# jgrodzki/radix_sort

Measured on AMD Instinct MI355X. Metric: Gkeys/sec (u64), higher is better.
Workload: dtype u64

## Files before the change

include/rsx.h:

```cpp
#ifndef RSX_H
#define RSX_H

#include <stddef.h>
#include <stdint.h>

#ifdef __cplusplus
extern "C" {
#endif

#define RSX_VERSION 200

enum {
    RSX_OK = 0,
    RSX_ERR_ARG = -1,
    RSX_ERR_UNSUPPORTED = -2,
    RSX_ERR_HIP = -3,
    RSX_ERR_NOMEM = -4,
    RSX_ERR_NODEVICE = -5,
    RSX_ERR_WORKSPACE = -6,
    RSX_ERR_INTERNAL = -7
};

enum {
    RSX_KEY_UNSIGNED = 0,
    RSX_KEY_SIGNED = 1,
    RSX_KEY_FLOAT = 2
};

#define RSX_MAX_ELEM_BYTES 32768u
typedef struct rsx_layout {
    uint32_t elem_bytes;
    uint32_t key_offset;
    uint32_t key_bytes;
    uint32_t key_kind;
} rsx_layout;

typedef struct rsx_ctx rsx_ctx;

int rsx_ctx_create(int device, rsx_ctx **out);
int rsx_ctx_destroy(rsx_ctx *ctx);
int rsx_ctx_reserve(rsx_ctx *ctx, size_t n, const rsx_layout *layout);
int rsx_ctx_check(rsx_ctx *ctx, void *stream);
enum {
    RSX_OPT_TILE_SCHEDULE = 1,
    RSX_OPT_RANKING = 2,
    RSX_OPT_STATUS_SCOPE = 3,
    RSX_OPT_XCD_MAJOR = 4,
    RSX_OPT_BYTE_COUNTING = 5,
    RSX_OPT_MAX_REGIONS = 6,
    RSX_OPT_HOT_LANES = 7,
    RSX_OPT_VERBOSE = 8,
    RSX_OPT_RANK_CHECK = 9,
    RSX_OPT_SMALL_SORT = 10,
    RSX_OPT_MID_SORT = 11      ,
    RSX_OPT_WIDE_SORT = 12,
    RSX_OPT_BUCKET_SKIP = 13,
    RSX_OPT_BUCKET_GROUP = 14
};
int rsx_ctx_set_option(rsx_ctx *ctx, int option, uint64_t value);
enum {
    RSX_INFO_RANK_ATOMIC = 1,
    RSX_INFO_L2_LOCAL = 2,
    RSX_INFO_NUM_CU = 3,
    RSX_INFO_DEVICE = 4,
    RSX_INFO_LAST_PASSES = 5,
    RSX_INFO_LAST_PAIRS = 6
};
int rsx_ctx_get_info(rsx_ctx *ctx, int what, uint64_t *out);
enum { RSX_PROF_HIST = 0, RSX_PROF_SCAN = 1, RSX_PROF_SWEEP = 2, RSX_PROF_OTHER = 3, RSX_PROF_KINDS = 4 };
int rsx_ctx_profile(rsx_ctx *ctx, int enable);
int rsx_ctx_profile_read(rsx_ctx *ctx, double *ms, uint64_t *launches);
const char *rsx_last_error(const rsx_ctx *ctx);
const char *rsx_strerror(int status);
int rsx_version(void);

int rsx_sort_device(rsx_ctx *ctx, void *d_data, void *d_tmp, size_t n, const rsx_layout *layout,
                    void *stream);

int rsx_sort_host(rsx_ctx *ctx, void *data, size_t n, const rsx_layout *layout);

int rsx_sort_segments_device(rsx_ctx *ctx, void *d_data, void *d_tmp, size_t n, const rsx_layout *layout,
                             const uint64_t *d_offsets, size_t nseg, uint64_t max_seg_len, void *stream);
int rsx_sort_rows_device(rsx_ctx *ctx, void *d_data, void *d_tmp, size_t rows, size_t row_len,
                         const rsx_layout *layout, void *stream);
#define RSX_SEG_CLASSES 2
int rsx_segment_caps(const rsx_layout *layout, uint32_t *caps);

enum { RSX_ORDER_ASCENDING = 0, RSX_ORDER_DESCENDING = 1 };

int rsx_sort_pairs_device(rsx_ctx *ctx, void *d_keys, void *d_values, size_t n, uint32_t key_bytes,
                          uint32_t key_kind, uint32_t value_bytes, int order, void *stream);
int rsx_argsort_device(rsx_ctx *ctx, const void *d_keys, void *d_index, size_t n, uint32_t key_bytes,
                       uint32_t key_kind, uint32_t index_bytes, int order, void *stream);
int rsx_ctx_reserve_pairs(rsx_ctx *ctx, size_t n, uint32_t key_bytes, uint32_t value_bytes);

int rsx_histogram_device(rsx_ctx *ctx, const void *d_src, size_t n, const rsx_layout *layout,
                         uint32_t digit, uint64_t *d_hist, void *stream);
int rsx_partition_device(rsx_ctx *ctx, const void *d_src, void *d_dst, size_t n,
                         const rsx_layout *layout, uint32_t digit, uint64_t *d_hist, void *stream);
int rsx_partition_count_device(rsx_ctx *ctx, const void *d_src, size_t n, const rsx_layout *layout, uint32_t digit,
                               uint32_t nsub, uint64_t *d_hist, void *stream);
int rsx_partition_scatter_device(rsx_ctx *ctx, const void *d_src, void *d_dst, size_t n, const rsx_layout *layout,
                                 uint32_t digit, uint32_t nsub, uint32_t k, void *stream);

int rsx_segmented_copy_device(rsx_ctx *ctx, const void *d_src, void *d_dst, uint32_t elem_bytes,
                              const uint64_t *d_src_off, const uint64_t *d_dst_off,
                              const uint64_t *d_len, uint32_t nseg, void *stream);

int rsx_bounds_device(rsx_ctx *ctx, const void *d_sorted, size_t n, const rsx_layout *layout,
                      const uint64_t *d_queries, uint32_t nq, uint64_t *d_out, void *stream);
// ... 36 lines not shown
```

radix_sort_amd/__init__.py:

```python
from .api import (PRIMITIVES, Context, RadixDigits, default_context, digits_of, radix_argsort, radix_sort, radix_sort_pairs,
                  radix_sort_rows, radix_sort_segments, radix_sort_sharded, segment_caps, tuple_of)
from ._lib import (GEN_CONSTANT, GEN_GEOMETRIC, GEN_PAYLOAD_ZERO, GEN_REVERSED, GEN_SORTED, GEN_STEP, GEN_UNIFORM,
                   GEN_ZIPF, INFO_L2_LOCAL, INFO_LAST_PAIRS, INFO_LAST_PASSES, INFO_RANK_ATOMIC, KEY_FLOAT, KEY_SIGNED, KEY_UNSIGNED, OPT_BYTE_COUNTING,
                   OPT_HOT_LANES, OPT_MAX_REGIONS, OPT_MID_SORT, OPT_WIDE_SORT, OPT_BUCKET_SKIP, OPT_BUCKET_GROUP, OPT_RANK_CHECK, OPT_RANKING, OPT_SMALL_SORT, OPT_STATUS_SCOPE, OPT_TILE_SCHEDULE, OPT_VERBOSE,
                   OPT_XCD_MAJOR, SHARD_EXCHANGE_FIRST, SHARD_SORT_FIRST, Layout, RsxError)

__all__ = ["radix_sort", "radix_sort_pairs", "radix_argsort", "radix_sort_segments", "radix_sort_rows", "segment_caps", "radix_sort_sharded", "RadixDigits", "PRIMITIVES", "tuple_of", "digits_of", "Context", "default_context",
           "Layout", "RsxError", "KEY_UNSIGNED", "KEY_SIGNED", "KEY_FLOAT", "GEN_UNIFORM", "GEN_ZIPF", "GEN_STEP",
           "GEN_SORTED", "GEN_REVERSED", "GEN_CONSTANT", "GEN_GEOMETRIC", "GEN_PAYLOAD_ZERO", "OPT_TILE_SCHEDULE",
           "OPT_RANKING", "OPT_STATUS_SCOPE", "OPT_XCD_MAJOR", "OPT_BYTE_COUNTING", "OPT_MAX_REGIONS", "OPT_HOT_LANES",
           "OPT_VERBOSE", "OPT_RANK_CHECK", "OPT_SMALL_SORT", "OPT_MID_SORT", "OPT_WIDE_SORT", "OPT_BUCKET_SKIP", "OPT_BUCKET_GROUP", "INFO_RANK_ATOMIC", "INFO_L2_LOCAL", "INFO_LAST_PASSES", "INFO_LAST_PAIRS", "SHARD_EXCHANGE_FIRST", "SHARD_SORT_FIRST"]
```

radix_sort_amd/_lib.py:

```python
from __future__ import annotations

import ctypes
import os

from . import _build

SYMBOLS = [
    "rsx_ctx_create", "rsx_ctx_destroy", "rsx_ctx_reserve", "rsx_ctx_check", "rsx_ctx_set_option", "rsx_ctx_get_info",
    "rsx_ctx_profile", "rsx_ctx_profile_read", "rsx_last_error",
    "rsx_strerror", "rsx_version", "rsx_sort_device", "rsx_sort_host", "rsx_histogram_device",
    "rsx_partition_device", "rsx_partition_count_device", "rsx_partition_scatter_device", "rsx_splitter_count_device",
    "rsx_splitter_pick_device", "rsx_segmented_copy_device", "rsx_bounds_device", "rsx_bounds_ranges_device", "rsx_sort_sharded",
    "rsx_sort_sharded_ex", "rsx_generate_device", "rsx_verify_device",
    "rsx_sort_segments_device", "rsx_sort_rows_device", "rsx_segment_caps",
    "rsx_sort_pairs_device", "rsx_argsort_device", "rsx_ctx_reserve_pairs",
]
SEG_CLASSES = 2

OK, ERR_ARG, ERR_UNSUPPORTED, ERR_HIP, ERR_NOMEM, ERR_NODEVICE, ERR_WORKSPACE, ERR_INTERNAL = 0, -1, -2, -3, -4, -5, -6, -7
KEY_UNSIGNED, KEY_SIGNED, KEY_FLOAT = 0, 1, 2
PROF_HIST, PROF_SCAN, PROF_SWEEP, PROF_OTHER, PROF_KINDS = 0, 1, 2, 3, 4
GEN_UNIFORM, GEN_ZIPF, GEN_STEP, GEN_SORTED, GEN_REVERSED, GEN_CONSTANT, GEN_GEOMETRIC = 0, 1, 2, 3, 4, 5, 6
GEN_PAYLOAD_ZERO = 0x100
(OPT_TILE_SCHEDULE, OPT_RANKING, OPT_STATUS_SCOPE, OPT_XCD_MAJOR, OPT_BYTE_COUNTING, OPT_MAX_REGIONS, OPT_HOT_LANES,
 OPT_VERBOSE, OPT_RANK_CHECK, OPT_SMALL_SORT, OPT_MID_SORT, OPT_WIDE_SORT, OPT_BUCKET_SKIP, OPT_BUCKET_GROUP) = 1, 2, 3, 4, 5, 6, 7, 8, 9, 10, 11, 12, 13, 14
INFO_RANK_ATOMIC, INFO_L2_LOCAL, INFO_NUM_CU, INFO_DEVICE, INFO_LAST_PASSES, INFO_LAST_PAIRS = 1, 2, 3, 4, 5, 6
ORDER_ASCENDING, ORDER_DESCENDING = 0, 1
SHARD_EXCHANGE_FIRST, SHARD_SORT_FIRST = 0, 1


class Layout(ctypes.Structure):
    _fields_ = [
        ("elem_bytes", ctypes.c_uint32),
        ("key_offset", ctypes.c_uint32),
        ("key_bytes", ctypes.c_uint32),
        ("key_kind", ctypes.c_uint32),
    ]

    def __repr__(self):
        return f"Layout(elem_bytes={self.elem_bytes}, key_offset={self.key_offset}, key_bytes={self.key_bytes}, key_kind={self.key_kind})"


class RsxError(RuntimeError):
    def __init__(self, status: int, msg: str):
        super().__init__(f"rsx status {status}: {msg}")
        self.status = status


_LIB = None


def lib_path() -> str:
    return os.environ.get("RSX_LIBRARY") or _build.LIB


def load():
    global _LIB
    if _LIB is not None:
        return _LIB
    try:
        import torch
    except ImportError:
        pass
    path = lib_path()
    if not os.path.exists(path):
        raise ImportError(
            f"{path} is missing: build it with `python -m radix_sort_amd._build` "
            "(needs hipcc); there is no CPU fallback for the sort path")
    L = ctypes.CDLL(path)
    vp, sz, lp = ctypes.c_void_p, ctypes.c_size_t, ctypes.POINTER(Layout)
    u32, u64, i = ctypes.c_uint32, ctypes.c_uint64, ctypes.c_int
    L.rsx_ctx_create.argtypes = [i, ctypes.POINTER(vp)]
    L.rsx_ctx_destroy.argtypes = [vp]
    L.rsx_ctx_reserve.argtypes = [vp, sz, lp]
    L.rsx_ctx_check.argtypes = [vp, vp]
    L.rsx_ctx_set_option.argtypes = [vp, i, u64]
    L.rsx_ctx_get_info.argtypes = [vp, i, ctypes.POINTER(ctypes.c_uint64)]
    L.rsx_ctx_profile.argtypes = [vp, i]
# ... 34 lines not shown
```

radix_sort_amd/csrc/rsx.hip:

```cpp
#include "rsx_internal.hpp"
#include "rsx_misc_kernels.hpp"
#include "rsx_any_kernels.hpp"

#include <cmath>

using namespace rsx;
using namespace rsxh;

namespace {

bool layout_ok(const rsx_layout* L, bool any_width = false) {
    if (!L) return false;
    const uint32_t kb = L->key_bytes;
    if (any_width ? (kb < 1 || kb > 16) : !(kb == 1 || kb == 2 || kb == 4 || kb == 8 || kb == 16)) return false;
    if (L->key_kind > RSX_KEY_FLOAT) return false;
    if (L->key_kind == RSX_KEY_FLOAT && !(kb == 4 || kb == 8)) return false;
    if (L->elem_bytes == 0 || (uint64_t)L->key_offset + kb > L->elem_bytes) return false;
    return true;
}
const EsLaunchers* launchers_for(uint32_t es) {
    switch (es) {
        case 1: return &es_launchers<1>();
        case 2: return &es_launchers<2>();
        case 4: return &es_launchers<4>();
// ... 760 lines not shown
        case RSX_OPT_TILE_SCHEDULE:
            if (value > 1) return fail(ctx, RSX_ERR_ARG, "RSX_OPT_TILE_SCHEDULE: 0 (roll call) or 1 (tickets)");
            flag(OPT_DYNAMIC_TILES, value == 1);
            return RSX_OK;
        case RSX_OPT_RANKING:
            if (value > 2) return fail(ctx, RSX_ERR_ARG, "RSX_OPT_RANKING: 0 (auto), 1 (ballots) or 2 (LDS atomics)");
            flag(OPT_BALLOT_RANKS, value == 1);
            flag(OPT_ATOMIC_RANKS, value == 2);
            return RSX_OK;
        case RSX_OPT_STATUS_SCOPE:
            if (value > 1) return fail(ctx, RSX_ERR_ARG, "RSX_OPT_STATUS_SCOPE: 0 (auto) or 1 (agent)");
            flag(OPT_AGENT_STATUS, value == 1);
            return RSX_OK;
        case RSX_OPT_XCD_MAJOR:
            if (value > 1) return fail(ctx, RSX_ERR_ARG, "RSX_OPT_XCD_MAJOR: 0 or 1");
            flag(OPT_NO_XCD_MAJOR, value == 0);
            return RSX_OK;
        case RSX_OPT_BYTE_COUNTING:
            if (value > 1) return fail(ctx, RSX_ERR_ARG, "RSX_OPT_BYTE_COUNTING: 0 or 1");
            flag(OPT_GENERAL_BYTES, value == 0);
            return RSX_OK;
        case RSX_OPT_MAX_REGIONS:
            if (value > (uint64_t)MAX_REGIONS) return fail(ctx, RSX_ERR_ARG, "RSX_OPT_MAX_REGIONS: 0 (default) .. 32");
            ctx->max_regions = (uint32_t)value;
            return RSX_OK;
        case RSX_OPT_HOT_LANES:
            if (value < 2 || value > 65) return fail(ctx, RSX_ERR_ARG, "RSX_OPT_HOT_LANES: 2 .. 65");
            ctx->hot_lanes = (uint32_t)value;
            return RSX_OK;
        case RSX_OPT_VERBOSE:
            flag(OPT_VERBOSE, value != 0);
            return RSX_OK;
        case RSX_OPT_RANK_CHECK:
            flag(OPT_RANK_CHECK, value != 0);
            return RSX_OK;
        case RSX_OPT_SMALL_SORT:
            if (value > 1) return fail(ctx, RSX_ERR_ARG, "RSX_OPT_SMALL_SORT: 0 or 1");
            flag(OPT_NO_SMALL_SORT, value == 0);
            return RSX_OK;
        case RSX_OPT_WIDE_SORT:
            if (value > 3) return fail(ctx, RSX_ERR_ARG, "RSX_OPT_WIDE_SORT: 0 (off), 1 (auto), 2 (always) or 3 (auto from 2^22 elements on)");
            ctx->wide_mode = (uint32_t)value;
            ctx->wide_skip = 0;
            if (ctx->host_err) host_word(ctx, HV_WIDE_HINT) = 0;
            return RSX_OK;
        case RSX_OPT_BUCKET_SKIP:
            if (value > 1) return fail(ctx, RSX_ERR_ARG, "RSX_OPT_BUCKET_SKIP: 0 or 1");
            ctx->bucket_no_skip = value == 0 ? 1u : 0u;
            return RSX_OK;
        case RSX_OPT_BUCKET_GROUP:
            if (value > 1) return fail(ctx, RSX_ERR_ARG, "RSX_OPT_BUCKET_GROUP: 0 or 1");
            ctx->bucket_group = (uint32_t)value;
            return RSX_OK;
        case RSX_OPT_MID_SORT:
            if (value > 3) return fail(ctx, RSX_ERR_ARG, "RSX_OPT_MID_SORT: 0 (off), 1 (forecast), 2 (always split) or 3 (always LSD passes)");
            flag(OPT_NO_MID_SORT, value == 0);
            ctx->mid_force = value >= 2 ? (uint32_t)value - 1u : 0u;
            return RSX_OK;
        default:
            return fail(ctx, RSX_ERR_ARG, "unknown option");
    }
} catch (...) {
    return RSX_ERR_NOMEM;
}

int rsx_ctx_get_info(rsx_ctx* ctx, int what, uint64_t* out) try {
    if (!ctx || !out) return RSX_ERR_ARG;
    std::lock_guard<std::mutex> lk(ctx->mu);
    DeviceGuard g(ctx->device);
    if (what == RSX_INFO_RANK_ATOMIC || what == RSX_INFO_L2_LOCAL) {
        int rc = ensure_aux(ctx, nullptr);
        if (rc) return rc;
    }
    switch (what) {
        case RSX_INFO_RANK_ATOMIC: *out = ctx->rank_atomic ? 1 : 0; return RSX_OK;
        case RSX_INFO_L2_LOCAL: *out = ctx->l2_local ? 1 : 0; return RSX_OK;
        case RSX_INFO_NUM_CU: *out = (uint64_t)ctx->num_cu; return RSX_OK;
        case RSX_INFO_DEVICE: *out = (uint64_t)ctx->device; return RSX_OK;
        case RSX_INFO_LAST_PASSES: {
            if (ctx->last_path == 6) {
                *out = (uint64_t)(ctx->last_sort_passes & 0xFFu) | (uint64_t)6 << 24;
                return RSX_OK;
            }
            *out = (uint64_t)ctx->last_path << 24 | (uint64_t)ctx->last_route << 28;
            if (!ctx->aux || ctx->last_sort_passes == 0) return RSX_OK;
            if (ctx->busy) RSX_HIP(hipEventSynchronize(ctx->last_event));
            uint64_t stat = 0, placed = 0;
            uint32_t path = ctx->last_path, passes = ctx->last_sort_passes;
            if (path == 5 && ctx->wide_buf) {
                uint32_t verdict = 0;
                RSX_HIP(hipMemcpy(&verdict, reinterpret_cast<char*>(ctx->wide_buf) + WIDE_PLAN_OFFSET, sizeof verdict, hipMemcpyDeviceToHost));
                if ((verdict & VERDICT_PATH_MASK) == VERDICT_HYBRID) passes = 2;
                else path = 0;
            }
            for (uint32_t p = 0; p < passes && p < (uint32_t)MAX_PASSES; ++p) {
                uint32_t mode = 0;
                RSX_HIP(hipMemcpy(&mode, reinterpret_cast<uint32_t*>(cb_of(ctx, ctx->cb_last) + CB_TICKETS) + (size_t)p * TICKET_WORDS + ROLL_MODE,
                                  sizeof mode, hipMemcpyDeviceToHost));
                stat += (mode == 1u || mode == 3u) ? 1u : 0u;
                placed += mode == 3u ? 1u : 0u;
            }
            *out = (uint64_t)passes | (stat << 8) | (placed << 16) | ((uint64_t)path << 24) | ((uint64_t)ctx->last_route << 28);
            return RSX_OK;
        }
        case RSX_INFO_LAST_PAIRS: *out = (uint64_t)ctx->last_pairs; return RSX_OK;
        default: return fail(ctx, RSX_ERR_ARG, "unknown info id");
// ... 910 lines not shown
```

radix_sort_amd/csrc/rsx_internal.hpp:

```cpp
#pragma once
#include "rsx_device.hpp"

#include <hip/hip_runtime.h>

#include <cstdio>
#include <cstdlib>
#include <cstring>
#include <mutex>
#include <new>
#include <algorithm>
#include <string>
#include <thread>
#include <utility>
#include <vector>

#include "../../include/rsx.h"

namespace rsxh {
using namespace rsx;

constexpr int MAX_PASSES = 16;
constexpr size_t J_BYTES = (size_t)J_REPL * MAX_REGIONS * RADIX * sizeof(uint64_t);
constexpr size_t TICKET_WORDS = ROLL_SHARDS + (size_t)ROLL_SHARD_COUNT * ROLL_SHARD_STRIDE;
constexpr uint32_t PART_MAX_SUB = 16;
constexpr uint32_t MID_MAX_REGIONS = 16;
constexpr size_t CB_TICKETS = 0;
constexpr size_t CB_JT = ((MAX_PASSES * TICKET_WORDS * 4 + 255) / 256) * 256;
constexpr size_t JT_BYTES = (size_t)J_REPL * MID_MAX_REGIONS * RADIX * sizeof(uint64_t);
constexpr size_t CB_J0 = CB_JT + JT_BYTES;
constexpr size_t CB_BYTES = CB_J0 + J_BYTES;
static_assert(CB_BYTES % 16 == 0, "control blocks are zeroed with 16-byte stores");
constexpr int CB_COUNT = 3;
constexpr size_t OFF_J1 = CB_COUNT * CB_BYTES;
constexpr size_t OFF_J2 = OFF_J1 + J_BYTES;
constexpr size_t OFF_PART_TICKETS = OFF_J2 + J_BYTES;
constexpr size_t OFF_BASE = OFF_PART_TICKETS + ((TICKET_WORDS * 4 + 255) / 256) * 256;
constexpr size_t OFF_FLAGS = OFF_BASE + 4096;
constexpr size_t OFF_DBG = OFF_FLAGS + 256;
constexpr size_t AUX_BYTES = OFF_DBG + 1024;
constexpr uint32_t HV_ERROR = 0, HV_MID_HINT = 8, HV_WIDE_HINT = 9;

enum : uint32_t {
    OPT_DYNAMIC_TILES = 1u << 0,
    OPT_BALLOT_RANKS = 1u << 1,
    OPT_ATOMIC_RANKS = 1u << 2,
    OPT_AGENT_STATUS = 1u << 3,
    OPT_NO_XCD_MAJOR = 1u << 4,
    OPT_GENERAL_BYTES = 1u << 5,
    OPT_VERBOSE = 1u << 6,
    OPT_RANK_CHECK = 1u << 7,
    OPT_NO_SMALL_SORT = 1u << 8,
    OPT_NO_MID_SORT = 1u << 9,
};

}

struct rsx_ctx {
    int device = 0;
    std::mutex mu;
    std::string err = "";
    void* status = nullptr;
    size_t status_bytes = 0;
    char* aux = nullptr;
    uint32_t* host_err = nullptr;
    uint32_t* host_err_dev = nullptr;
    void* host_buf[2] = {nullptr, nullptr};
    size_t host_bytes = 0;
    hipStream_t copy_stream = nullptr;
    void* pinned[4] = {nullptr, nullptr, nullptr, nullptr};
    hipEvent_t copy_event[4] = {nullptr, nullptr, nullptr, nullptr};
    uint32_t wide_skip = 0;
    char* wide_buf = nullptr;
    uint32_t wide_mode = 1;
    std::vector<const void*> lds_attr;
    uint64_t wide_tried_sig = 0, wide_refused_sig = 0;
    uint32_t bucket_no_skip = 0;
    uint32_t bucket_group = 1;
    uint32_t* ovf16 = nullptr;
    unsigned long long* part_J = nullptr;
    hipStream_t shard_stream = nullptr;
    uint64_t* shard_q = nullptr;
    uint64_t* shard_out = nullptr;
    uint64_t* shard_hist = nullptr;
    uint64_t* shard_host = nullptr;
    std::vector<uint64_t> shard_stage;
    int num_cu = 256;
    uint32_t last_path = 0;
    uint32_t last_sort_passes = 0;
    uint32_t last_route = 0;
    char* any_buf = nullptr;
    size_t any_bytes = 0;
    uint32_t last_pairs = 0;
    uint64_t cb_used[2][2] = {{0, 0}, {0, 0}};
    uint32_t cb_alt = 0;
    uint32_t cb_last = 0;
    bool cb_dirty = false;
    uint32_t mid_choice = 0;
    uint32_t mid_force = 0;
    uint32_t mid_cooldown = 0;
    bool rank_atomic = false;
    bool l2_local = false;
    uint32_t hot_lanes = 16;
    uint32_t options = 0;
    uint32_t max_regions = 0;
    uint32_t dbg = 0;
    hipStream_t last_stream = nullptr;
    hipEvent_t last_event = nullptr;
    bool busy = false;
    bool prof = false;
    std::vector<std::pair<hipEvent_t, hipEvent_t>> prof_pending[RSX_PROF_KINDS];
    std::vector<std::pair<hipEvent_t, hipEvent_t>> prof_free;
    double prof_ms[RSX_PROF_KINDS] = {0, 0, 0, 0};
    uint64_t prof_n[RSX_PROF_KINDS] = {0, 0, 0, 0};
    std::vector<float> prof_each;
};

namespace rsxh {

struct SortRun {
    uint32_t cb = 0;
    CleanList clean = {{nullptr, nullptr, nullptr}, {0, 0, 0}};
    Gate gate = {nullptr, 0, 0};
    const DigitSpec* spec_dev = nullptr;
    uint32_t* tickets_override = nullptr;
};
struct SweepPass {
    uint32_t index;
    bool last;
    uint32_t mid;
};
// ... 200 lines not shown
```

radix_sort_amd/csrc/rsx_launch_impl.hpp:

```cpp
#pragma once
#include <cstdlib>
#include "rsx_internal.hpp"
#include "rsx_small_kernel.hpp"
#include "rsx_mid_kernels.hpp"
#include "rsx_segment_kernels.hpp"

#ifndef RSX_HIST_BLOCKS_PER_CU
#define RSX_HIST_BLOCKS_PER_CU 8
#endif

namespace rsxh {

inline uint32_t rank_atomic_of(const rsx_ctx* ctx) { return (ctx->rank_atomic && !(ctx->options & OPT_BALLOT_RANKS)) ? 1u : 0u; }
constexpr CleanList CLEAN_NONE = {{nullptr, nullptr, nullptr}, {0, 0, 0}};

inline uint64_t hist_blocks_per_region(const rsx_ctx* ctx, const RegionGeom& g) {
    const uint64_t per_block = 512ull * 16;
    uint64_t bpr = ((1ull << g.region_shift) + per_block - 1) / per_block;
    const uint64_t cap = ((uint64_t)ctx->num_cu * RSX_HIST_BLOCKS_PER_CU + g.num_regions - 1) / g.num_regions;
    if (bpr > cap) bpr = cap;
    return bpr == 0 ? 1 : bpr;
}
template <int ES, bool FLT>
int launch_hist_t(rsx_ctx* ctx, SortRun& run, const void* src, const RegionGeom& g, const rsx_layout* L, uint32_t digit,
// ... 333 lines not shown
            auto kern = rsx_count16top_kernel<ES, true>;
            ensure_lds(ctx, reinterpret_cast<const void*>(kern), 131072);
            hipLaunchKernelGGL(kern, dim3(parts), dim3(1024), 131072, st, static_cast<const Elem<ES>*>(src), (uint64_t)n, plan, make_xform(L), P,
                               ctx->ovf16, region_shift, k);
        } else {
            auto kern = rsx_count16top_kernel<ES, false>;
            ensure_lds(ctx, reinterpret_cast<const void*>(kern), 131072);
            hipLaunchKernelGGL(kern, dim3(parts), dim3(1024), 131072, st, static_cast<const Elem<ES>*>(src), (uint64_t)n, plan, make_xform(L), P,
                               ctx->ovf16, region_shift, k);
        }
        RSX_HIP(hipGetLastError());
        return RSX_OK;
    }
}

template <int ES>
int launch_marginal16(rsx_ctx* ctx, SortRun& run, const uint32_t* P, uint32_t parts, uint32_t k, const RegionGeom& g, unsigned long long* J,
                      unsigned long long* jclear, hipStream_t st) {
    const uint64_t zero16_n = status_rows(g) * RADIX * (status32(g) ? 4u : 8u) / 16u;
    uint32_t grid = (uint32_t)ctx->num_cu * 8u;
    if (grid < parts) grid = parts;
    LaunchTimer lt(ctx, RSX_PROF_HIST, st);
    hipLaunchKernelGGL(rsx_marginal16_kernel<ES>, dim3(grid), dim3(256), 0, st, P, parts, k, g, J, jclear, status32(g) ? 1u : 0u,
                       static_cast<uint4*>(ctx->status), zero16_n, run.clean, run.gate);
    RSX_HIP(hipGetLastError());
    run.clean = CLEAN_NONE;
    return RSX_OK;
}

template <int ES>
int launch_bucket16(rsx_ctx* ctx, const SortRun& run, void* data, void* scratch, size_t n, const rsx_layout* L, const uint64_t* starts,
                    const WidePlan* plan, hipStream_t st) {
    if constexpr (ES < 4) {
        return fail(ctx, RSX_ERR_INTERNAL, "launch_bucket16: narrow elements");
    } else {
        constexpr int KPT = bucket_kpt_for(ES);
        if (L->key_bytes < 4) return fail(ctx, RSX_ERR_INTERNAL, "launch_bucket16: key width out of range");
        SmallArgs a = small_args(ctx, L, L->key_bytes - 2, L->key_bytes, false);
        a.src = data;
        a.data = data;
        a.cap = bucket_cap(ES);
        LaunchTimer lt(ctx, RSX_PROF_OTHER, st);
        const uint64_t avg = (uint64_t)n / 65536u;
        const uint32_t gs = group_shift(ctx, n, L);
        const Gate base = run.gate;
        auto go = [&](auto wgc, auto kc, uint32_t form, uint32_t group_shift) {
            constexpr int WGS = decltype(wgc)::value;
            constexpr int K = decltype(kc)::value;
            SmallArgs b = a;
            b.group_shift = group_shift;
            if (group_shift) b.passes = L->key_bytes;
            static_assert(cape<ES, K, WGS>() == bucket_cape(ES, K, WGS), "host and device agree on what a workgroup holds");
            const size_t lds = (size_t)cape<ES, K, WGS>() * ES + (WGS / 64) * RADIX * bucket_cnt_bytes() + 64 + 3 * RADIX * sizeof(uint32_t);
            auto kern = rsx_bucket16_kernel<ES, K, WGS>;
            ensure_lds(ctx, reinterpret_cast<const void*>(kern), lds);
            int per_cu = (int)((size_t)163840 / lds);
            if (per_cu < 1) per_cu = 1;
            if (per_cu > 4 * RSX_B16_WAVES(WGS) * 64 / WGS) per_cu = 4 * RSX_B16_WAVES(WGS) * 64 / WGS;
            const Gate g{base.word, VERDICT_PATH_MASK | VERDICT_FORM_MASK, VERDICT_HYBRID | form};
            hipLaunchKernelGGL(kern, dim3((uint32_t)(ctx->num_cu * per_cu)), dim3(WGS), lds, st, b, starts, scratch, plan, g);
        };
        using std::integral_constant;
        constexpr int KBIG = wide_kpt_for(ES);
        if (gs >= 2) go(integral_constant<int, 512>{}, integral_constant<int, KPT>{}, VERDICT_GROUPS, gs);
        if (avg <= (uint64_t)256 * KPT) go(integral_constant<int, 256>{}, integral_constant<int, KPT>{}, VERDICT_WG256, 0);
        if (avg <= (uint64_t)512 * KPT) go(integral_constant<int, 512>{}, integral_constant<int, KPT>{}, VERDICT_WG512, 0);
        const bool big_form = KBIG != KPT && wide_big_form(ES, n);
        if (big_form) go(integral_constant<int, 1024>{}, integral_constant<int, KBIG>{}, VERDICT_WG1024, 0);
        else go(integral_constant<int, 1024>{}, integral_constant<int, KPT>{}, VERDICT_WG1024, 0);
        {
            constexpr int KMED = medium_kpt_for(ES);
            const size_t lds = (size_t)cape<ES, KMED, 1024>() * ES + 16 * RADIX * bucket_cnt_bytes() + 64 + 3 * RADIX * sizeof(uint32_t);
            auto kern = rsx_bucket16_medium_kernel<ES, KMED, 1024>;
            ensure_lds(ctx, reinterpret_cast<const void*>(kern), lds);
            const Gate g{base.word, VERDICT_PATH_MASK | VERDICT_MEDIUM, VERDICT_HYBRID | VERDICT_MEDIUM};
            hipLaunchKernelGGL(kern, dim3((uint32_t)ctx->num_cu), dim3(1024), lds, st, a, starts, scratch, plan, (uint32_t)(256 * KPT), (uint32_t)(512 * KPT),
                               (uint32_t)(big_form ? cape<ES, KBIG, 1024>() : cape<ES, KPT, 1024>()), g);
        }
        RSX_HIP(hipGetLastError());
        return RSX_OK;
    }
}

template <int ES>
int launch_segcopy(rsx_ctx* ctx, const void* src, void* dst, const uint64_t* so, const uint64_t* dof,
                   const uint64_t* len, uint32_t nseg, hipStream_t st) {
    const uint32_t bps = 8;
    hipLaunchKernelGGL((rsx_segcopy_kernel<ES>), dim3(nseg * bps), dim3(256), 0, st,
                       static_cast<const Elem<ES>*>(src), static_cast<Elem<ES>*>(dst), so, dof, len, nseg, bps);
    RSX_HIP(hipGetLastError());
    return RSX_OK;
}

template <int ES>
int launch_segment_sort(rsx_ctx* ctx, void* data, void* tmp, size_t n, const rsx_layout* L, const uint64_t* offsets, uint64_t nseg,
                        uint64_t row_len, uint64_t max_len, uint32_t* launched, hipStream_t st) {
    constexpr int KPT = bucket_kpt_for(ES);
    constexpr uint32_t CAP0 = cape<ES, KPT, 256>(), CAP1 = cape<ES, KPT, 1024>();
    static_assert(CAP0 == segment_cap(ES, 0) && CAP1 == segment_cap(ES, 1), "host and device agree on what a workgroup holds");
    if (L->key_bytes > 16) return fail(ctx, RSX_ERR_INTERNAL, "launch_segment_sort: key width out of range");
    SmallArgs a = small_args(ctx, L, L->key_bytes, L->key_bytes, true);
    if (L->key_bytes < 6) a.no_skip = 1u;
    SmallArgs am = a;
    am.map_load = am.map_store = 0;
    for (uint32_t d = 0; d < L->key_bytes; ++d) am.spec[d] = make_spec(L, d);
    SegArgs s;
    std::memset(&s, 0, sizeof s);
// ... 50 lines not shown
```

radix_sort_amd/csrc/rsx_small_kernel.hpp:

```cpp
#pragma once
#include "rsx_device.hpp"

namespace rsx {

struct SmallArgs {
    const void* src;
    void* data;
    uint32_t n;
    uint32_t passes;
    uint32_t rank_atomic;
    uint32_t map_load;
    uint32_t map_store;
    DigitSpec spec[16];
    KeyXform xf;
    const uint32_t* top_tot;
    uint32_t cap;
    uint32_t no_skip;
    uint32_t group_shift;
    uint32_t key_offset, key_bytes;
    uint32_t* hint;
};

struct PassPlan {
    uint32_t first, end;
// ... 396 lines not shown
    for (int w = 0; w < ES / 4; ++w) {
        mm.hi[w] = pp.mask[w];
        mm.lo[w] = pp.low[w];
    }
    return mend_listed<ES>(reinterpret_cast<Elem<ES>*>(smem), mend_count<ES, KPT, WG>(smem), s_flag, n, (uint32_t)WG, ties, mm) != 0;
}
template <int ES, int KPT, int WG>
__device__ __forceinline__ void local_store_regs(const SmallArgs& a, Elem<ES>* __restrict__ dst, const uint32_t n, Elem<ES> (&x)[KPT]) {
#pragma unroll
    for (int j = 0; j < KPT; ++j) {
        const uint32_t i = (uint32_t)j * WG + threadIdx.x;
        if (i < n) {
            if (a.map_store) key_map<ES, true>(x[j], a.xf);
            dst[i] = x[j];
        }
    }
}

template <int ES, int KPT, int WG>
__device__ __forceinline__ bool local_finish(const SmallArgs& a, Elem<ES>* __restrict__ dst, const uint32_t n, unsigned char* smem, const PassPlan& pp,
                                             uint32_t* s_flag) {
    Elem<ES> x[KPT];
    uint32_t ties;
    if (!local_check<ES, KPT, WG>(pp, n, smem, x, ties)) {
        local_store_regs<ES, KPT, WG>(a, dst, n, x);
        return true;
    }
    if (!local_mend_listed<ES, KPT, WG>(n, smem, pp, s_flag, ties)) return false;
    local_store<ES, KPT, WG>(a, dst, n, smem);
    return true;
}

template <int ES, int KPT, int WG>
__device__ __forceinline__ void local_sort_skip(const SmallArgs& a, const Elem<ES>* __restrict__ src, Elem<ES>* __restrict__ dst, const uint32_t n,
                                                unsigned char* smem, PassPlan& pp, uint32_t* s_flag) {
    using E = Elem<ES>;
    E e[KPT];
    local_load<ES, KPT, WG>(a, src, n, e);
    local_passes<ES, KPT, WG>(a, e, n, smem, pp.first, pp.end);
    if (pp.first == 0) {
        local_store<ES, KPT, WG>(a, dst, n, smem);
    } else if (!local_finish<ES, KPT, WG>(a, dst, n, smem, pp, s_flag)) {
        pp.first = 0;
        const uint32_t kp = (n + WG - 1) / WG, seg = (threadIdx.x >> 6) * (WAVE * kp) + (threadIdx.x & 63u);
#pragma unroll
        for (int j = 0; j < KPT; ++j)
            if ((uint32_t)j < kp) e[j] = reinterpret_cast<const E*>(smem)[seg + (uint32_t)j * WAVE];
        __syncthreads();
        local_passes<ES, KPT, WG>(a, e, n, smem, 0, pp.end);
        local_store<ES, KPT, WG>(a, dst, n, smem);
    }
}

template <int ES, int KPT>
__global__ __launch_bounds__(512) void rsx_small_sort_kernel(const SmallArgs a) {
    extern __shared__ __attribute__((aligned(16))) unsigned char smem[];
    local_sort<ES, KPT, 512>(a, static_cast<const Elem<ES>*>(a.src), static_cast<Elem<ES>*>(a.data), a.n, smem);
}

template <int ES, int KPT, int WG>
__global__ __launch_bounds__(WG) void rsx_bucket_sort_kernel(const SmallArgs a) {
    extern __shared__ __attribute__((aligned(16))) unsigned char smem[];
    uint64_t* s_red = reinterpret_cast<uint64_t*>(smem);
    const uint32_t tid = threadIdx.x, v = blockIdx.x;
    uint64_t c = 0;
    if (tid < RADIX) {
        c = a.top_tot[tid];
        if (tid == v) s_red[4] = c;
        if (v == 0) {
            uint64_t big = c;
#pragma unroll
            for (int o = 32; o > 0; o >>= 1) {
                const uint64_t y = __shfl_xor(big, o);
                big = y > big ? y : big;
            }
            if ((tid & 63u) == 0u) s_red[5 + (tid >> 6)] = big;
        }
        uint64_t below = tid < v ? c : 0ull;
#pragma unroll
        for (int o = 32; o > 0; o >>= 1) below += __shfl_xor(below, o);
        if ((tid & 63u) == 0u) s_red[tid >> 6] = below;
    }
    __syncthreads();
    const uint64_t start = s_red[0] + s_red[1] + s_red[2] + s_red[3];
    const uint64_t count = s_red[4];
    if (v == 0 && tid == 0) {
        uint64_t big = s_red[5];
        for (int w = 1; w < 4; ++w) big = s_red[5 + w] > big ? s_red[5 + w] : big;
        __hip_atomic_store(a.hint, big <= (uint64_t)a.cap / 4 ? 1u : big <= (uint64_t)a.cap ? 3u : 2u, __ATOMIC_RELAXED, __HIP_MEMORY_SCOPE_SYSTEM);
    }
    __syncthreads();
    if (count == 0) return;
    if (count > (uint64_t)cape<ES, KPT, WG>()) {
        big_bucket_sort<ES, KPT, WG>(a, const_cast<Elem<ES>*>(static_cast<const Elem<ES>*>(a.src)) + start,
                                     static_cast<Elem<ES>*>(a.data) + start, (uint32_t)count, smem);
        return;
    }
    if constexpr (ES < 8) {
        local_sort<ES, KPT, WG>(a, static_cast<const Elem<ES>*>(a.src) + start, static_cast<Elem<ES>*>(a.data) + start, (uint32_t)count, smem);
    } else {
        PassPlan pp;
        pp.end = a.passes;
        pp.first = a.no_skip ? 0u : first_digit_for((uint32_t)count, 8u * a.passes, a.passes);
        pp.set_masks(a.key_offset, a.key_bytes);
        uint32_t* s_flag = reinterpret_cast<uint32_t*>(reinterpret_cast<typename WaveCnt<ES>::T*>(smem + (size_t)cape<ES, KPT, WG>() * sizeof(Elem<ES>)) + (WG / WAVE) * RADIX) + (WG / WAVE);
        local_sort_skip<ES, KPT, WG>(a, static_cast<const Elem<ES>*>(a.src) + start, static_cast<Elem<ES>*>(a.data) + start, (uint32_t)count, smem, pp,
                                     s_flag);
    }
}

template <int ES, int KPT, int WG>
__global__ __launch_bounds__(WG, RSX_B16_WAVES(WG)) void rsx_bucket16_kernel(const SmallArgs a, const uint64_t* __restrict__ starts, void* scratch,
                                                                         const WidePlan* __restrict__ plan, Gate gate) {
    extern __shared__ __attribute__((aligned(16))) unsigned char smem[];
    if (!gate_open(gate)) return;
    using E = Elem<ES>;
    constexpr int NWAVE = WG / WAVE;
    uint32_t* s_flag = reinterpret_cast<uint32_t*>(reinterpret_cast<typename WaveCnt<ES>::T*>(smem + (size_t)cape<ES, KPT, WG>() * sizeof(E)) + NWAVE * RADIX) + NWAVE;
    const uint32_t gs = a.group_shift != 0 ? plan->group_shift : 0;
    const bool medium = (plan->verdict & VERDICT_MEDIUM) != 0;
    PassPlan pp;
    pp.end = gs == 0 ? plan->pass_end : plan->group_end;
    if (pp.end == 0) {
        if (a.map_store) {
            const uint64_t n = starts[65536];
            E* data = static_cast<E*>(a.data);
            for (uint64_t i = (uint64_t)blockIdx.x * WG + threadIdx.x; i < n; i += (uint64_t)gridDim.x * WG) {
                E x = data[i];
                key_map<ES, true>(x, a.xf);
                data[i] = x;
            }
        }
        return;
    }
    const uint32_t b_lo = plan->window_top - 15u;
    const uint32_t end_sub = pp.end;
    if (gs != 0) pp.end = (b_lo + gs + 7u) / 8u;
    {
        const uint64_t big = (uint64_t)plan->scan_max << gs;
        const uint32_t m = big < (uint64_t)cape<ES, KPT, WG>() ? (uint32_t)big : cape<ES, KPT, WG>();
        pp.first = a.no_skip ? 0u : first_digit_for(m, b_lo + gs, pp.end);
    }
    pp.set_masks(a.key_offset, a.key_bytes);
    for (uint32_t g = blockIdx.x; g < (65536u >> gs); g += gridDim.x) {
        const uint32_t b0 = g << gs;
        const uint64_t gstart = starts[b0];
        const uint64_t gcount = starts[b0 + (1u << gs)] - gstart;
        if (gcount == 0) continue;
        const bool whole = gs == 0 || gcount <= (uint64_t)cape<ES, KPT, WG>();
        const uint32_t nsub = whole ? 1u : 1u << gs;
        for (uint32_t sub = 0; sub < nsub; ++sub) {
            uint64_t start = gstart, count = gcount;
            if (!whole) {
                start = starts[b0 + sub];
                count = starts[b0 + sub + 1] - start;
            }
            if (count != 0) {
                E* bucket = static_cast<E*>(a.data) + start;
                if (count <= (uint64_t)cape<ES, KPT, WG>()) {
                    const uint32_t first = pp.first, end = pp.end;
                    if (!whole) {
                        pp.first = 0;
                        pp.end = end_sub;
                    }
                    local_sort_skip<ES, KPT, WG>(a, bucket, bucket, (uint32_t)count, smem, pp, s_flag);
                    if (!whole) {
                        pp.first = first;
                        pp.end = end;
                    }
                } else if (!medium) {
                    big_bucket_sort<ES, KPT, WG>(a, bucket, static_cast<E*>(scratch) + start, (uint32_t)count, smem);
                }
            }
            __syncthreads();
        }
    }
}

template <int ES, int KPT, int WG>
__global__ __launch_bounds__(WG, RSX_B16_WAVES(WG)) void rsx_bucket16_medium_kernel(const SmallArgs a, const uint64_t* __restrict__ starts, void* scratch,
                                                                                const WidePlan* __restrict__ plan, uint32_t cap256, uint32_t cap512,
                                                                                uint32_t cap1024, Gate gate) {
    extern __shared__ __attribute__((aligned(16))) unsigned char smem[];
    __shared__ uint32_t s_part[2];
    if (!gate_open(gate)) return;
    using E = Elem<ES>;
    constexpr int NWAVE = WG / WAVE;
    constexpr uint32_t CAPE = cape<ES, KPT, WG>();
    uint32_t* s_flag = reinterpret_cast<uint32_t*>(reinterpret_cast<typename WaveCnt<ES>::T*>(smem + (size_t)CAPE * sizeof(E)) + NWAVE * RADIX) + NWAVE;
    const uint32_t tid = threadIdx.x;
    const uint32_t form = plan->verdict & VERDICT_FORM_MASK;
    const uint64_t handled = form == VERDICT_WG256 ? cap256 : form == VERDICT_WG1024 ? cap1024 : cap512;
    const uint32_t end = plan->pass_end;
    if (end == 0) return;
    const uint32_t b_lo = plan->window_top - 15u;
    for (uint32_t b = blockIdx.x; b < 65536u; b += gridDim.x) {
        const uint64_t start = starts[b];
        const uint64_t count = starts[b + 1] - start;
        if (count <= handled) continue;
        E* bucket = static_cast<E*>(a.data) + start;
        E* scr = static_cast<E*>(scratch) + start;
        uint32_t k = 0;
        while (k < 8u && (count >> k) > (uint64_t)CAPE * 6u / 10u) ++k;
        if (k > b_lo) k = b_lo;
        const bool split = !(k == 0 || (count >> k) > (uint64_t)CAPE || count > 0xFFFFFFFFull);
        uint32_t kmask = 0, part_start = 0, part_count = (uint32_t)count;
        PassPlan pp;
        pp.end = end;
        pp.first = 0;
        if (split) {
            DigitSpec sp{};
            const uint32_t ebit = 8u * a.key_offset + b_lo - k;
            sp.word = ebit >> 5;
            sp.shift = ebit & 31u;
            kmask = (1u << k) - 1u;
            part_start = part_count = 0;
            const uint32_t km = kmask;
            stream_pass<ES, KPT, WG>(a, bucket, scr, (uint32_t)count, smem, [&](const E& x) { return elem_digit_any<ES>(x, sp) & km; }, false, part_start,
// ... 32 lines not shown
```

Before: 67.97.

## Prefetch next bucket into LDS during store in bucket16 kernel

Adds a prefetching variant of the 16-bit bucket sort kernel that issues asynchronous global-to-LDS loads of the next bucket this workgroup will handle. The loads are interleaved with the store of the current sorted bucket, and the next local sort reads its input from LDS instead of global memory. The goal is to hide global load latency between consecutive buckets. In exchange it adds inline assembly, alignment and bounds conditions, and a waitcnt on every bucket. The variant is on by default for 1024-thread workgroups with 8- or 16-byte elements.

```diff
diff --git a/include/rsx.h b/include/rsx.h
--- a/include/rsx.h
+++ b/include/rsx.h
@@ -55,7 +55,8 @@
     RSX_OPT_MID_SORT = 11      ,
     RSX_OPT_WIDE_SORT = 12,
     RSX_OPT_BUCKET_SKIP = 13,
-    RSX_OPT_BUCKET_GROUP = 14
+    RSX_OPT_BUCKET_GROUP = 14,
+    RSX_OPT_BUCKET_PREFETCH = 15
 };
 int rsx_ctx_set_option(rsx_ctx *ctx, int option, uint64_t value);
 enum {
diff --git a/radix_sort_amd/__init__.py b/radix_sort_amd/__init__.py
--- a/radix_sort_amd/__init__.py
+++ b/radix_sort_amd/__init__.py
@@ -2,11 +2,11 @@
                   radix_sort_rows, radix_sort_segments, radix_sort_sharded, segment_caps, tuple_of)
 from ._lib import (GEN_CONSTANT, GEN_GEOMETRIC, GEN_PAYLOAD_ZERO, GEN_REVERSED, GEN_SORTED, GEN_STEP, GEN_UNIFORM,
                    GEN_ZIPF, INFO_L2_LOCAL, INFO_LAST_PAIRS, INFO_LAST_PASSES, INFO_RANK_ATOMIC, KEY_FLOAT, KEY_SIGNED, KEY_UNSIGNED, OPT_BYTE_COUNTING,
-                   OPT_HOT_LANES, OPT_MAX_REGIONS, OPT_MID_SORT, OPT_WIDE_SORT, OPT_BUCKET_SKIP, OPT_BUCKET_GROUP, OPT_RANK_CHECK, OPT_RANKING, OPT_SMALL_SORT, OPT_STATUS_SCOPE, OPT_TILE_SCHEDULE, OPT_VERBOSE,
+                   OPT_HOT_LANES, OPT_MAX_REGIONS, OPT_MID_SORT, OPT_WIDE_SORT, OPT_BUCKET_SKIP, OPT_BUCKET_GROUP, OPT_BUCKET_PREFETCH, OPT_RANK_CHECK, OPT_RANKING, OPT_SMALL_SORT, OPT_STATUS_SCOPE, OPT_TILE_SCHEDULE, OPT_VERBOSE,
                    OPT_XCD_MAJOR, SHARD_EXCHANGE_FIRST, SHARD_SORT_FIRST, Layout, RsxError)
 
 __all__ = ["radix_sort", "radix_sort_pairs", "radix_argsort", "radix_sort_segments", "radix_sort_rows", "segment_caps", "radix_sort_sharded", "RadixDigits", "PRIMITIVES", "tuple_of", "digits_of", "Context", "default_context",
            "Layout", "RsxError", "KEY_UNSIGNED", "KEY_SIGNED", "KEY_FLOAT", "GEN_UNIFORM", "GEN_ZIPF", "GEN_STEP",
            "GEN_SORTED", "GEN_REVERSED", "GEN_CONSTANT", "GEN_GEOMETRIC", "GEN_PAYLOAD_ZERO", "OPT_TILE_SCHEDULE",
            "OPT_RANKING", "OPT_STATUS_SCOPE", "OPT_XCD_MAJOR", "OPT_BYTE_COUNTING", "OPT_MAX_REGIONS", "OPT_HOT_LANES",
-           "OPT_VERBOSE", "OPT_RANK_CHECK", "OPT_SMALL_SORT", "OPT_MID_SORT", "OPT_WIDE_SORT", "OPT_BUCKET_SKIP", "OPT_BUCKET_GROUP", "INFO_RANK_ATOMIC", "INFO_L2_LOCAL", "INFO_LAST_PASSES", "INFO_LAST_PAIRS", "SHARD_EXCHANGE_FIRST", "SHARD_SORT_FIRST"]
+           "OPT_VERBOSE", "OPT_RANK_CHECK", "OPT_SMALL_SORT", "OPT_MID_SORT", "OPT_WIDE_SORT", "OPT_BUCKET_SKIP", "OPT_BUCKET_GROUP", "OPT_BUCKET_PREFETCH", "INFO_RANK_ATOMIC", "INFO_L2_LOCAL", "INFO_LAST_PASSES", "INFO_LAST_PAIRS", "SHARD_EXCHANGE_FIRST", "SHARD_SORT_FIRST"]
diff --git a/radix_sort_amd/_lib.py b/radix_sort_amd/_lib.py
--- a/radix_sort_amd/_lib.py
+++ b/radix_sort_amd/_lib.py
@@ -23,7 +23,8 @@
 GEN_UNIFORM, GEN_ZIPF, GEN_STEP, GEN_SORTED, GEN_REVERSED, GEN_CONSTANT, GEN_GEOMETRIC = 0, 1, 2, 3, 4, 5, 6
 GEN_PAYLOAD_ZERO = 0x100
 (OPT_TILE_SCHEDULE, OPT_RANKING, OPT_STATUS_SCOPE, OPT_XCD_MAJOR, OPT_BYTE_COUNTING, OPT_MAX_REGIONS, OPT_HOT_LANES,
- OPT_VERBOSE, OPT_RANK_CHECK, OPT_SMALL_SORT, OPT_MID_SORT, OPT_WIDE_SORT, OPT_BUCKET_SKIP, OPT_BUCKET_GROUP) = 1, 2, 3, 4, 5, 6, 7, 8, 9, 10, 11, 12, 13, 14
+ OPT_VERBOSE, OPT_RANK_CHECK, OPT_SMALL_SORT, OPT_MID_SORT, OPT_WIDE_SORT, OPT_BUCKET_SKIP, OPT_BUCKET_GROUP,
+ OPT_BUCKET_PREFETCH) = 1, 2, 3, 4, 5, 6, 7, 8, 9, 10, 11, 12, 13, 14, 15
 INFO_RANK_ATOMIC, INFO_L2_LOCAL, INFO_NUM_CU, INFO_DEVICE, INFO_LAST_PASSES, INFO_LAST_PAIRS = 1, 2, 3, 4, 5, 6
 ORDER_ASCENDING, ORDER_DESCENDING = 0, 1
 SHARD_EXCHANGE_FIRST, SHARD_SORT_FIRST = 0, 1
diff --git a/radix_sort_amd/csrc/rsx.hip b/radix_sort_amd/csrc/rsx.hip
--- a/radix_sort_amd/csrc/rsx.hip
+++ b/radix_sort_amd/csrc/rsx.hip
@@ -836,6 +836,10 @@
             if (value > 1) return fail(ctx, RSX_ERR_ARG, "RSX_OPT_BUCKET_GROUP: 0 or 1");
             ctx->bucket_group = (uint32_t)value;
             return RSX_OK;
+        case RSX_OPT_BUCKET_PREFETCH:
+            if (value > 1) return fail(ctx, RSX_ERR_ARG, "RSX_OPT_BUCKET_PREFETCH: 0 or 1");
+            ctx->bucket_prefetch = (uint32_t)value;
+            return RSX_OK;
         case RSX_OPT_MID_SORT:
             if (value > 3) return fail(ctx, RSX_ERR_ARG, "RSX_OPT_MID_SORT: 0 (off), 1 (forecast), 2 (always split) or 3 (always LSD passes)");
             flag(OPT_NO_MID_SORT, value == 0);
diff --git a/radix_sort_amd/csrc/rsx_internal.hpp b/radix_sort_amd/csrc/rsx_internal.hpp
--- a/radix_sort_amd/csrc/rsx_internal.hpp
+++ b/radix_sort_amd/csrc/rsx_internal.hpp
@@ -76,6 +76,7 @@
     uint64_t wide_tried_sig = 0, wide_refused_sig = 0;
     uint32_t bucket_no_skip = 0;
     uint32_t bucket_group = 1;
+    uint32_t bucket_prefetch = 1;
     uint32_t* ovf16 = nullptr;
     unsigned long long* part_J = nullptr;
     hipStream_t shard_stream = nullptr;
diff --git a/radix_sort_amd/csrc/rsx_launch_impl.hpp b/radix_sort_amd/csrc/rsx_launch_impl.hpp
--- a/radix_sort_amd/csrc/rsx_launch_impl.hpp
+++ b/radix_sort_amd/csrc/rsx_launch_impl.hpp
@@ -409,7 +409,11 @@
             if (group_shift) b.passes = L->key_bytes;
             static_assert(cape<ES, K, WGS>() == bucket_cape(ES, K, WGS), "host and device agree on what a workgroup holds");
             const size_t lds = (size_t)cape<ES, K, WGS>() * ES + (WGS / 64) * RADIX * bucket_cnt_bytes() + 64 + 3 * RADIX * sizeof(uint32_t);
-            auto kern = rsx_bucket16_kernel<ES, K, WGS>;
+            constexpr bool CAN_PF = WGS == 1024 && (ES == 8 || ES == 16);
+            auto kern = rsx_bucket16_kernel<ES, K, WGS, false>;
+            if constexpr (CAN_PF) {
+                if (ctx->bucket_prefetch) kern = rsx_bucket16_kernel<ES, K, WGS, true>;
+            }
             ensure_lds(ctx, reinterpret_cast<const void*>(kern), lds);
             int per_cu = (int)((size_t)163840 / lds);
             if (per_cu < 1) per_cu = 1;
diff --git a/radix_sort_amd/csrc/rsx_small_kernel.hpp b/radix_sort_amd/csrc/rsx_small_kernel.hpp
--- a/radix_sort_amd/csrc/rsx_small_kernel.hpp
+++ b/radix_sort_amd/csrc/rsx_small_kernel.hpp
@@ -472,6 +472,137 @@
     }
 }
 
+__device__ __forceinline__ uint32_t uniform32(const uint32_t v) { return (uint32_t)__builtin_amdgcn_readfirstlane((int)v); }
+__device__ __forceinline__ uint64_t uniform64(const uint64_t v) { return (uint64_t)uniform32((uint32_t)v) | ((uint64_t)uniform32((uint32_t)(v >> 32)) << 32); }
+template <int ES, int KPT, int WG>
+__device__ __forceinline__ void tile_prefetch(const unsigned char* __restrict__ src_, const uint32_t pieces_, unsigned char* smem) {
+    static_assert(ES == 8 || ES == 16, "16-byte pieces of whole elements");
+    const unsigned char* src = reinterpret_cast<const unsigned char*>(uniform64(reinterpret_cast<uintptr_t>(src_)));
+    const uint32_t pieces = uniform32(pieces_);
+    constexpr int ROUNDS = (KPT * ES + 15) / 16;
+    const uint32_t lane = threadIdx.x & 63u;
+    const uint32_t wbase = (uint32_t)__builtin_amdgcn_readfirstlane((int)(threadIdx.x & ~63u));
+#pragma unroll
+    for (int r = 0; r < ROUNDS; ++r) {
+        const uint32_t c0 = (uint32_t)r * WG + wbase;
+        if (c0 + lane < pieces)
+            __builtin_amdgcn_global_load_lds((const __attribute__((address_space(1))) void*)(src + (uint32_t)(16u * (c0 + lane))),
+                                             (__attribute__((address_space(3))) void*)(smem + 16u * c0), 16, 0, 0);
+    }
+}
+template <int ES, int KPT, int WG>
+__device__ __forceinline__ void local_load_lds(const unsigned char* smem, const uint32_t par, const uint32_t n, Elem<ES> (&e)[KPT]) {
+    const Elem<ES>* s_img = reinterpret_cast<const Elem<ES>*>(smem) + par;
+    const uint32_t tid = threadIdx.x, lane = tid & 63u, wave = tid >> 6;
+    const uint32_t kp = (n + WG - 1) / WG;
+    const uint32_t seg = wave * (WAVE * kp) + lane;
+#pragma unroll
+    for (int j = 0; j < KPT; ++j) {
+        e[j] = Elem<ES>{};
+        if ((uint32_t)j < kp) {
+            const uint32_t p = seg + (uint32_t)j * WAVE;
+            if (p < n) e[j] = s_img[p];
+        }
+    }
+}
+#ifndef RSX_PF_UNROLL
+#define RSX_PF_UNROLL 1
+#endif
+static_assert(RSX_PF_UNROLL == 1 || RSX_PF_UNROLL == 2 || RSX_PF_UNROLL == 4, "rounds per trip of local_store_pf");
+template <int ES, int KPT, int WG>
+__device__ __forceinline__ void local_store_pf(const SmallArgs& a, Elem<ES>* __restrict__ dst, const uint32_t n, unsigned char* smem,
+                                               const unsigned char* __restrict__ next_src, const uint32_t next_pieces) {
+    static_assert(ES == 8 || ES == 16, "16-byte pieces of whole elements");
+    using E = Elem<ES>;
+    constexpr uint32_t PER = 16 / ES;
+    constexpr uint32_t LANES = WAVE / PER;
+    const unsigned char* src = reinterpret_cast<const unsigned char*>(uniform64(reinterpret_cast<uintptr_t>(next_src)));
+    const uint32_t pieces = uniform32(next_pieces);
+    const uint32_t lane = threadIdx.x & 63u;
+    const uint32_t lds0 = (uint32_t)reinterpret_cast<uintptr_t>((__attribute__((address_space(3))) unsigned char*)smem);
+    const uint32_t top = n > pieces * PER ? n : pieces * PER;
+    typedef uint32_t u32xe __attribute__((ext_vector_type(ES / 4)));
+    constexpr uint32_t U = RSX_PF_UNROLL;
+    for (uint32_t i0 = uniform32(threadIdx.x & ~63u); i0 < top; i0 += U * WG) {
+        u32xe v[U];
+#pragma unroll
+        for (uint32_t u = 0; u < U; ++u) {
+            const uint32_t i = i0 + u * WG + lane;
+            v[u] = u32xe{};
+            if (i < n) {
+                if constexpr (ES == 8) asm volatile("ds_read_b64 %0, %1" : "=v"(v[u]) : "v"(lds0 + i * 8u) : "memory");
+                else asm volatile("ds_read_b128 %0, %1" : "=v"(v[u]) : "v"(lds0 + i * 16u) : "memory");
+            }
+        }
+        if constexpr (U == 1) asm volatile("s_waitcnt lgkmcnt(0)" : "+v"(v[0]) : : "memory");
+        else if constexpr (U == 2) asm volatile("s_waitcnt lgkmcnt(0)" : "+v"(v[0]), "+v"(v[1]) : : "memory");
+        else asm volatile("s_waitcnt lgkmcnt(0)" : "+v"(v[0]), "+v"(v[1]), "+v"(v[2]), "+v"(v[3]) : : "memory");
+#pragma unroll
+        for (uint32_t u = 0; u < U; ++u) {
+            const uint32_t i = i0 + u * WG + lane;
+            if (i < n) {
+                E x;
+#pragma unroll
+                for (int w = 0; w < ES / 4; ++w) x.w[w] = v[u][w];
+                if (a.map_store) key_map<ES, true>(x, a.xf);
+                dst[i] = x;
+            }
+        }
+#pragma unroll
+        for (uint32_t u = 0; u < U; ++u) {
+            const uint32_t c0 = (i0 + u * WG) / PER;
+            if (lane < LANES && c0 + lane < pieces)
+                __builtin_amdgcn_global_load_lds((const __attribute__((address_space(1))) void*)(src + (uint32_t)(16u * (c0 + lane))),
+                                                 (__attribute__((address_space(3))) void*)(smem + 16u * c0), 16, 0, 0);
+        }
+    }
+}
+#ifndef RSX_PF_REGS
+#define RSX_PF_REGS 0
+#endif
+template <int ES, int KPT, int WG>
+__device__ __forceinline__ bool local_finish_pf(const SmallArgs& a, Elem<ES>* __restrict__ dst, const uint32_t n, unsigned char* smem, const PassPlan& pp,
+                                                uint32_t* s_flag, const unsigned char* __restrict__ next_src, const uint32_t next_pieces) {
+    Elem<ES> x[KPT];
+    uint32_t ties;
+#if RSX_PF_REGS
+    if (!local_check<ES, KPT, WG>(pp, n, smem, x, ties)) {
+        tile_prefetch<ES, KPT, WG>(next_src, next_pieces, smem);
+        local_store_regs<ES, KPT, WG>(a, dst, n, x);
+        return true;
+    }
+    if (!local_mend_listed<ES, KPT, WG>(n, smem, pp, s_flag, ties)) return false;
+#else
+    if (local_check<ES, KPT, WG>(pp, n, smem, x, ties) && !local_mend_listed<ES, KPT, WG>(n, smem, pp, s_flag, ties)) return false;
+#endif
+    local_store_pf<ES, KPT, WG>(a, dst, n, smem, next_src, next_pieces);
+    return true;
+}
+template <int ES, int KPT, int WG>
+__device__ __forceinline__ bool local_sort_skip_pf(const SmallArgs& a, const Elem<ES>* __restrict__ src, Elem<ES>* __restrict__ dst, const uint32_t n,
+                                                   unsigned char* smem, PassPlan& pp, uint32_t* s_flag, const bool have, const uint32_t par,
+                                                   const unsigned char* __restrict__ next_src, const uint32_t next_pieces) {
+    using E = Elem<ES>;
+    E e[KPT];
+    if (have) local_load_lds<ES, KPT, WG>(smem, par, n, e);
+    else local_load<ES, KPT, WG>(a, src, n, e);
+    local_passes<ES, KPT, WG>(a, e, n, smem, pp.first, pp.end);
+    if (pp.first == 0) {
+        local_store<ES, KPT, WG>(a, dst, n, smem);
+        return false;
+    }
+    if (local_finish_pf<ES, KPT, WG>(a, dst, n, smem, pp, s_flag, next_src, next_pieces)) return next_pieces != 0;
+    pp.first = 0;
+    const uint32_t kp = (n + WG - 1) / WG, seg = (threadIdx.x >> 6) * (WAVE * kp) + (threadIdx.x & 63u);
+#pragma unroll
+    for (int j = 0; j < KPT; ++j)
+        if ((uint32_t)j < kp) e[j] = reinterpret_cast<const E*>(smem)[seg + (uint32_t)j * WAVE];
+    __syncthreads();
+    local_passes<ES, KPT, WG>(a, e, n, smem, 0, pp.end);
+    local_store<ES, KPT, WG>(a, dst, n, smem);
+    return false;
+}
+
 template <int ES, int KPT>
 __global__ __launch_bounds__(512) void rsx_small_sort_kernel(const SmallArgs a) {
     extern __shared__ __attribute__((aligned(16))) unsigned char smem[];
@@ -529,7 +660,7 @@
     }
 }
 
-template <int ES, int KPT, int WG>
+template <int ES, int KPT, int WG, bool PF = false>
 __global__ __launch_bounds__(WG, RSX_B16_WAVES(WG)) void rsx_bucket16_kernel(const SmallArgs a, const uint64_t* __restrict__ starts, void* scratch,
                                                                          const WidePlan* __restrict__ plan, Gate gate) {
     extern __shared__ __attribute__((aligned(16))) unsigned char smem[];
@@ -562,6 +693,8 @@
         pp.first = a.no_skip ? 0u : first_digit_for(m, b_lo + gs, pp.end);
     }
     pp.set_masks(a.key_offset, a.key_bytes);
+    [[maybe_unused]] bool have = false;
+    [[maybe_unused]] uint32_t par = 0;
     for (uint32_t g = blockIdx.x; g < (65536u >> gs); g += gridDim.x) {
         const uint32_t b0 = g << gs;
         const uint64_t gstart = starts[b0];
@@ -583,7 +716,33 @@
                         pp.first = 0;
                         pp.end = end_sub;
                     }
-                    local_sort_skip<ES, KPT, WG>(a, bucket, bucket, (uint32_t)count, smem, pp, s_flag);
+                    if constexpr (PF) {
+                        const unsigned char* nsrc = nullptr;
+                        uint32_t npieces = 0, npar = 0;
+                        const uint32_t g2 = g + gridDim.x;
+                        if (whole && pp.first != 0 && g2 < (65536u >> gs)) {
+                            const uint64_t s2 = uniform64(starts[g2 << gs]), c2 = uniform64(starts[(g2 + 1u) << gs]) - s2;
+                            const E* b2 = static_cast<const E*>(a.data) + s2;
+                            if constexpr (ES == 8) {
+                                npar = (uint32_t)(reinterpret_cast<uintptr_t>(b2) >> 3) & 1u;
+                                const uint64_t slots = c2 + npar;
+                                if (c2 != 0 && slots <= (uint64_t)cape<ES, KPT, WG>() && s2 + c2 + (slots & 1u) <= uniform64(starts[65536])) {
+                                    nsrc = reinterpret_cast<const unsigned char*>(b2 - npar);
+                                    npieces = (uint32_t)((slots + 1u) >> 1);
+                                }
+                            } else {
+                                if (c2 != 0 && c2 <= (uint64_t)cape<ES, KPT, WG>() && (reinterpret_cast<uintptr_t>(b2) & 15u) == 0) {
+                                    nsrc = reinterpret_cast<const unsigned char*>(b2);
+                                    npieces = (uint32_t)c2;
+                                }
+                            }
+                        }
+                        have = local_sort_skip_pf<ES, KPT, WG>(a, bucket, bucket, (uint32_t)count, smem, pp, s_flag, have, par, nsrc, npieces);
+                        par = npar;
+                        if (have) asm volatile("s_waitcnt vmcnt(0)" ::: "memory");
+                    } else {
+                        local_sort_skip<ES, KPT, WG>(a, bucket, bucket, (uint32_t)count, smem, pp, s_flag);
+                    }
                     if (!whole) {
                         pp.first = first;
                         pp.end = end;
```

Result: slower. 64.53 (-5.1%).
